# sruckh/echo-tts

Measured on AMD Instinct MI355X. Metric: audio-sec/sec/GPU @ seq_len=640, 40 steps, CFG(text=3, spk=8); 1/2/4/8 GPU, higher is better.
Workload: dtype bf16; 1 GPU; C2: 48 utterance(s)/step/GPU (24 per sampler call, 2 HIP stream(s)), seq_len=640, 40 Euler steps (20 CFG x3 rows + 20 x1 row), cfg_text=3.0 cfg_spk=8.0, text 436 tokens padded to 768, one speaker latent (1,2560,80) encoded per call and shared by its rows, EchoDiT bf16 + Fish S1-DAC decode fp32, random weights; parallelism=dp1 (independent utterances, weight broadcast only)

## Files before the change

### echo-tts_amd/_lib.py

```python
from __future__ import annotations

import ctypes as C
import os

HERE = os.path.dirname(os.path.abspath(__file__))
LIB_PATH = os.environ.get("ECHO_LIB_PATH") or os.path.join(HERE, "libechohip.so")

ECHO_F32, ECHO_BF16 = 0, 1
ABI_VERSION = 8

c_i64 = C.c_int64
vp = C.c_void_p


class EchoConfig(C.Structure):
    _fields_ = [
        ("precision", C.c_int),
        ("latent_size", C.c_int), ("model_size", C.c_int), ("num_layers", C.c_int), ("num_heads", C.c_int),
        ("intermediate_size", C.c_int),
        ("norm_eps", C.c_float),
        ("text_vocab_size", C.c_int), ("text_model_size", C.c_int), ("text_num_layers", C.c_int),
        ("text_num_heads", C.c_int), ("text_intermediate_size", C.c_int),
        ("speaker_patch_size", C.c_int), ("speaker_model_size", C.c_int), ("speaker_num_layers", C.c_int),
        ("speaker_num_heads", C.c_int), ("speaker_intermediate_size", C.c_int),
# ... 71 lines not shown


SIGNATURES = {
    "echo_abi_version": (C.c_int, []),
    "echo_last_error": (C.c_char_p, [vp]),
    "echo_ctx_create": (C.c_int, [C.POINTER(EchoConfig), C.c_int, C.POINTER(vp)]),
    "echo_ctx_destroy": (None, [vp]),
    "echo_load_tensor": (C.c_int, [vp, C.c_char_p, vp, C.c_int, C.c_int, C.POINTER(c_i64), C.c_int]),
    "echo_finalize_dit": (C.c_int, [vp, vp]),
    "echo_finalize_dac": (C.c_int, [vp, vp]),
    "echo_set_rope_table": (C.c_int, [vp, vp, C.c_int]),
    "echo_set_ae_rope_table": (C.c_int, [vp, vp, C.c_int]),
    "echo_encode_text": (C.c_int, [vp, vp, vp, C.POINTER(C.c_int32), C.c_int, C.c_int, vp]),
    "echo_encode_speaker": (C.c_int, [vp, vp, vp, C.POINTER(C.c_int32), C.c_int, C.c_int, vp]),
    "echo_encode_latent_prefix": (C.c_int, [vp, vp, C.c_int, C.c_int, C.c_long, vp]),
    "echo_scale_speaker_kv": (C.c_int, [vp, C.c_float, C.c_int, vp]),
    "echo_dit_forward": (C.c_int, [vp, vp, vp, C.c_int, C.c_int, C.c_int, C.c_int, C.c_int, C.POINTER(C.c_int32),
                                   C.POINTER(C.c_int32), vp, vp]),
    "echo_dit_forward_t": (C.c_int, [vp, vp, vp, C.c_int, C.POINTER(C.c_int32), C.c_int, C.c_int, C.c_int, C.c_int, C.c_int,
                                     C.POINTER(C.c_int32), C.POINTER(C.c_int32), vp, vp]),
    "echo_sample_euler": (C.c_int, [vp, C.POINTER(EchoSamplerParams), vp, vp, vp]),
    "echo_dac_decode": (C.c_int, [vp, vp, C.c_int, C.c_float, vp, vp]),
    "echo_dac_decode_zq": (C.c_int, [vp, vp, C.c_int, vp, vp]),
    "echo_dac_decode_batch": (C.c_int, [vp, vp, C.c_int, C.c_int, C.c_float, vp, c_i64, vp]),
    "echo_set_pca": (C.c_int, [vp, vp, vp, C.c_int, vp]),
    "echo_dac_hop": (C.c_int, [vp]),
    "echo_finalize_dac_encoder": (C.c_int, [vp, vp]),
    "echo_dac_encode": (C.c_int, [vp, vp, C.c_long, vp, vp, vp, vp]),
    "echo_set_pca_encode": (C.c_int, [vp, vp, vp, C.c_float, C.c_int, vp]),
    "echo_op_gemm": (C.c_int, [C.c_int, C.POINTER(EchoGemmDesc), vp]),
    "echo_op_quant_rows_fp8": (C.c_int, [vp, c_i64, vp, c_i64, vp, C.c_int, C.c_int, vp]),
    "echo_op_norm_adaln_fp8": (C.c_int, [vp, c_i64, vp, c_i64, vp, C.c_int, C.c_int, C.c_float, vp, vp, vp]),
    "echo_op_presplit_weights": (C.c_int, [vp, c_i64, c_i64, vp]),
    "echo_op_pack_rows": (C.c_int, [vp, C.c_int, c_i64, vp, C.c_int, c_i64, C.c_int, C.c_int, C.c_int, C.c_int, vp]),
    "echo_op_attention_bf16": (C.c_int, [C.POINTER(EchoAttnDesc), vp]),
    "echo_op_attention_bf16_len": (C.c_int, [C.POINTER(EchoAttnDesc), vp, vp]),
    "echo_op_norm": (C.c_int, [C.c_int, C.c_int, vp, c_i64, vp, c_i64, C.c_int, C.c_int, C.c_float, vp, vp, vp]),
    "echo_op_headnorm_rope": (C.c_int, [C.c_int, vp, c_i64, c_i64, C.c_int, C.c_int, C.c_int, C.c_int, vp, c_i64, C.c_float,
                                        C.c_int, C.c_int, vp, C.c_int, C.c_int, vp]),
    "echo_op_transpose_heads": (C.c_int, [C.c_int, vp, c_i64, vp, c_i64, c_i64, C.c_int, C.c_int, C.c_int, C.c_int, vp]),
    "echo_debug_get_kv": (C.c_int, [vp, C.c_int, C.c_int, vp, vp, C.POINTER(C.c_int), C.POINTER(C.c_int)]),
    "echo_debug_corrupt_tile": (C.c_int, [vp, C.c_int]),
    "echo_op_resample": (C.c_int, [vp, c_i64, vp, C.c_int, C.c_int, C.c_int, C.c_int, vp, c_i64, vp]),
    "echo_voice_capture": (C.c_int, [vp, C.POINTER(vp), vp]),
    "echo_voice_bind": (C.c_int, [vp, vp, vp]),
    "echo_sample_euler_items": (C.c_int, [vp, C.POINTER(EchoSamplerParams), C.POINTER(EchoSamplerItem), vp, vp, vp]),
    "echo_dit_forward_pos": (C.c_int, [vp, vp, vp, C.c_int, C.POINTER(C.c_int32), C.c_int, C.c_int, C.c_int, C.POINTER(C.c_int32), C.c_int,
                                       C.POINTER(C.c_int32), C.POINTER(C.c_int32), vp, vp]),
    "echo_sample_euler_items_pos": (C.c_int, [vp, C.POINTER(EchoSamplerParams), C.POINTER(EchoSamplerItem), C.POINTER(C.c_int32), vp, vp, vp]),
    "echo_dit_forward_len": (C.c_int, [vp, vp, vp, C.c_int, C.POINTER(C.c_int32), C.c_int, C.c_int, C.c_int, C.POINTER(C.c_int32),
                                       C.POINTER(C.c_int32), C.c_int, C.POINTER(C.c_int32), C.POINTER(C.c_int32), vp, vp]),
    "echo_sample_euler_items_len": (C.c_int, [vp, C.POINTER(EchoSamplerParams), C.POINTER(EchoSamplerItem), C.POINTER(C.c_int32),
                                              C.POINTER(C.c_int32), vp, vp, vp]),
    "echo_scale_speaker_kv_items": (C.c_int, [vp, C.POINTER(C.c_float), C.POINTER(C.c_int32), C.c_int, vp]),
    "echo_voice_bind_items": (C.c_int, [vp, C.POINTER(vp), C.c_int, vp]),
    "echo_voice_bytes": (c_i64, [vp]),
    "echo_voice_destroy": (None, [vp]),
    "echo_dac_decode_tail": (C.c_int, [vp, vp, C.c_int, C.c_int, C.c_float, vp, vp]),
    "echo_workspace_bytes": (c_i64, [vp]),
    "echo_fp8_calibrate": (C.c_int, [vp, C.c_int]),
    "echo_fp8_calibration": (C.c_int, [vp, C.POINTER(C.c_float), C.c_int]),
    "echo_fp8_set_static_scales": (C.c_int, [vp, C.POINTER(C.c_float), C.c_int]),
    "echo_reserve_workspace": (C.c_int, [vp, C.c_int, C.c_int, C.c_int, C.c_int, C.c_int]),
    "echo_op_find_flattening_point": (C.c_int, [vp, c_i64, C.c_int, C.c_int, C.c_int, C.c_int, C.c_float, C.c_float, vp, vp]),
    "echo_op_trailing_quiet": (C.c_int, [C.POINTER(vp), C.POINTER(c_i64), C.c_int, C.c_int, C.c_float, vp, vp]),
    "echo_op_assemble_chunks": (C.c_int, [C.POINTER(vp), C.POINTER(c_i64), C.POINTER(c_i64), C.POINTER(c_i64), C.POINTER(C.c_int32),
# ... 37 lines not shown
```

### echo-tts_amd/build.py

```python
from __future__ import annotations

import os
import shutil
import subprocess
import sys

HERE = os.path.dirname(os.path.abspath(__file__))
CSRC = os.path.join(HERE, "csrc")
LIB = os.path.join(HERE, "libechohip.so")
SOURCES = ["gemm_pp.hip", "gemm.hip", "gemm_f32.hip", "attention.hip", "elementwise.hip", "dac.hip", "postproc.hip", "engine.hip"]
EXTRA_FLAGS = {"attention.hip": ["-fno-slp-vectorize"]}
COMMON_FLAGS = ["-ffp-contract=off"]


def _hipcc() -> str:
    for c in (os.environ.get("HIPCC"), "/opt/rocm/bin/hipcc", shutil.which("hipcc")):
        if c and os.path.exists(c):
            return c
    raise RuntimeError("hipcc not found (ROCm toolchain required)")


def needs_build() -> bool:
    if not os.path.exists(LIB):
        return True
    t = os.path.getmtime(LIB)
    deps = [os.path.join(CSRC, f) for f in os.listdir(CSRC)] + [os.path.join(HERE, "..", "include", "echo_hip.h")]
    return any(os.path.getmtime(d) > t for d in deps)


def build(force: bool = False, verbose: bool = True) -> str:
    if not force and not needs_build():
        return LIB
    objs = []
    os.makedirs(os.path.join(HERE, "build"), exist_ok=True)
    procs = []
    for src in SOURCES:
        obj = os.path.join(HERE, "build", src.replace(".hip", ".o"))
        cmd = [_hipcc(), "--offload-arch=gfx950", "-O3", "-std=c++17", "-fPIC"] + COMMON_FLAGS + EXTRA_FLAGS.get(src, []) + ["-c", os.path.join(CSRC, src), "-o", obj]
        procs.append((src, subprocess.Popen(cmd, stdout=subprocess.PIPE, stderr=subprocess.STDOUT, text=True)))
        objs.append(obj)
    for src, p in procs:
        out, _ = p.communicate()
        if p.returncode != 0:
# ... 13 lines not shown
```

### echo-tts_amd/csrc/common.h

```cpp
#pragma once
#include <hip/hip_runtime.h>
#include <stdint.h>
#include <string.h>
#include <atomic>
#include <string>

inline hipError_t ensure_dyn_lds(const void* kern, int bytes, std::atomic<unsigned long long>& done) {
  int dev = 0;
  hipError_t e = hipGetDevice(&dev);
  if (e != hipSuccess) return e;
  const unsigned long long bit = 1ull << (dev & 63);
  if (done.load(std::memory_order_acquire) & bit) return hipSuccess;
  e = hipFuncSetAttribute(kern, hipFuncAttributeMaxDynamicSharedMemorySize, bytes);
  if (e == hipSuccess) done.fetch_or(bit, std::memory_order_release);
  return e;
}

typedef uint16_t bf16_t;
typedef __attribute__((ext_vector_type(8))) short bf16x8;
typedef __attribute__((ext_vector_type(4))) short bf16x4;
typedef __attribute__((ext_vector_type(4))) float f32x4;
typedef __attribute__((ext_vector_type(4))) int i32x4;
typedef __attribute__((ext_vector_type(8))) int i32x8;
typedef __attribute__((ext_vector_type(16))) float f32x16;
// ... 74 lines not shown
  int nbatch, nbi;
  long a_bo, a_bi, w_bo, w_bi, c_bo, c_bi;
  float acc_scale;
  const void* bias; long bias_bo, bias_bi; int vec_mod;
  float div;
  int act;
  const void* colscale;
  const void* res; long ldres, res_bo, res_bi;
  const void* snake_alpha;
  int store_main;
  int swiglu;
  int cfg;
  int ksplit;
  void* ws; long ws_bytes;
  int split3;
  int w_presplit;
  float a_scale_const;
  void* c8; long c8_ld; float c8_inv;
  int pp_gn;
  int snake_fast;
  void* sink;
  int qkv_mode, qkv_D, qkv_S, rope_heads, pos0;
  int qkv_gate_act;
  float qk_eps;
  int rope_mod;
  const void* qk_w; const void* rope;
  void* vt; long vt_ld, vt_row_stride;
  int fp8; const float* a_scale; const float* w_scale;
};
int gemm_tile_m(int cfg);
int gemm_num_cfgs();
void gemm_args_init(GemmArgs* g);
template <typename T> hipError_t launch_gemm_nt(const GemmArgs& g, hipStream_t st);

struct AttnSeg {
  const bf16_t* K; long k_ld, k_row_stride, k_head_stride;
  const bf16_t* Vt; long vt_ld, vt_row_stride, vt_head_stride;
  const int* nkeys;
  const float* bias; long bias_row_stride;
  int kv_mod;
};
struct AttnArgs {
  const bf16_t* Q; long q_ld, q_row_stride;
  bf16_t* O; long o_ld, o_row_stride;
  const bf16_t* G; long g_ld, g_row_stride;
  int g_act;
  int S, H, rows;
  int nseg; AttnSeg seg[4];
  int causal;
  float scale;
  void* prof;
  int* redo;
  const int* redo_filter;
  int q_block0;
  int redo_nb;
  int q128;
  uint8_t* O8; long o8_ld, o8_row_stride; float o8_inv;
  const int* qlen;
};
inline long attn_redo_words(int rows, int H, int S) { return (long)rows * H * ((S + 127) / 128); }
hipError_t launch_attention_bf16(const AttnArgs& a, hipStream_t st);

enum NormMode { NORM_ADALN = 0, NORM_RMS_W = 1, NORM_AE_RMS = 2, NORM_LAYER = 3 };
template <typename T>
hipError_t launch_norm(int mode, const T* x, long ldx, T* y, long ldy, int rows, int D, float eps,
                       const T* w0, const T* w1, hipStream_t st);
// ... 106 lines not shown
```

### echo-tts_amd/csrc/engine.hip

```cpp
#include "common.h"
#include "../../include/echo_hip.h"

#include <dlfcn.h>

#include <cmath>
#include <cstdio>
#include <cstdlib>
#include <map>
#include <memory>
#include <mutex>
#include <string>
#include <vector>

namespace {

thread_local std::string g_create_error;

struct Plan { int cfg = 0, ksplit = 1; };
std::map<int, std::map<std::vector<long>, Plan>> g_plans;
std::mutex g_plans_mu;

inline long rup(long x, long m) { return (x + m - 1) / m * m; }

std::string plan_file_path() {
// ... 1762 lines not shown
        for (auto& ru : Bk.ru) {
          CK(launch_presplit_w(ru.w7, rup(Bk.co, 128), 7L * Bk.co, st));
          CK(launch_presplit_w(ru.w1, rup(Bk.co, 128), Bk.co, st));
        }
      }
    }
    }
    CK(hipStreamSynchronize(st));
    drop_raw({"quantizer.", "decoder."});
    dac_ready = true;
    return ECHO_OK;
  }

  bool dac_split3 = getenv("ECHO_DAC_EXACT_FP32") ? atoi(getenv("ECHO_DAC_EXACT_FP32")) == 0 : true;
  bool dac_fast_sin = getenv("ECHO_DAC_FAST_SIN") ? atoi(getenv("ECHO_DAC_FAST_SIN")) != 0 : true;
  DevBuf b_sink;
  template <typename X>
  int frun(const GemmArgs& g_in, hipStream_t st) {
    GemmArgs g = g_in;
    g.split3 = sizeof(X) == 4 && dac_split3 ? 1 : 0;
    if (sizeof(X) == 2) g.w_presplit = 0;
    if (!b_sink.p) CK(b_sink.reserve(262144));
    g.sink = b_sink.p;
    g.snake_fast = dac_fast_sin ? 1 : 0;
    if constexpr (sizeof(X) == 2) {
      const bool big = (long)g.M * g.Npad >= 256L * 256 * 64;
      g.cfg = !big ? 0 : g.N % 192 == 0 && g.N % 256 != 0 ? 8 : g.N % 96 == 0 && g.N % 128 != 0 ? 9 : g.N % 256 > 0 && g.N % 256 <= 128 ? 3 : 2;
      g.ksplit = 1;
    } else {
      CKI(plan_gemm<X>(g, st));
    }
    return run_planned<X>(g, st, false);
  }
  template <typename X>
  static GemmArgs FG(const X* A, long lda, const X* W, long ldw, X* C, long ldc, long M, int N, int K) {
    GemmArgs g;
    gemm_args_init(&g);
    g.A = A; g.lda = lda; g.W = W; g.ldw = ldw; g.C = C; g.ldc = ldc; g.M = (int)M; g.N = N; g.K = K;
    g.Npad = (int)rup(N, 128);
    return g;
  }

  int set_pca(const float* w, const float* mean, int on_device, hipStream_t st) override {
    if (!dac_ready) return fail("echo_finalize_dac was not called");
    const int C = cfg.dac_latent_dim, Lz = cfg.latent_size;
    const hipMemcpyKind kind = on_device ? hipMemcpyDeviceToDevice : hipMemcpyHostToDevice;
    CK(hipMemcpy2DAsync(pca_w, pca_kpad * sizeof(float), w, Lz * sizeof(float), Lz * sizeof(float), C, kind, st));
    CK(hipMemcpyAsync(pca_b, mean, C * sizeof(float), kind, st));
    CK(hipStreamSynchronize(st));
    pca_set = true;
    return ECHO_OK;
  }
  bool pca_set = false;
  int dac_decode(const float* lat, int Tn, float latent_scale, float* wav, hipStream_t st) override {
    if (!pca_set) return fail("echo_set_pca was not called");
    return dac_run(lat, nullptr, Tn, latent_scale, wav, st);
  }
  int dac_decode_zq(const float* z, int Tn, float* wav, hipStream_t st) override { return dac_run(nullptr, z, Tn, 1.0f, wav, st); }
  int dac_decode_tail(const float* lat, int Tn, int f0, float latent_scale, float* wav, hipStream_t st) override {
    if (!pca_set) return fail("echo_set_pca was not called");
    if (f0 < 0 || f0 >= Tn) return fail("bad first frame");
    return dac_run(lat, nullptr, Tn, latent_scale, wav, st, f0);
  }

  template <typename X>
  int dac_transformer(std::vector<DacLayerT<X>>& layers, X* x, int Tn, int C, int nh, int hd, int ff, int window, X* xn_buf,
// ... 380 lines not shown
    if (!front)
    for (auto& U : dups) {
      { GemmArgs g = FG(cur, C, U.w, C, other, (long)U.f * C, rows, U.f * C, C); g.bias = U.b; g.vec_mod = C; CKI(frun<T>(g, st)); }
      rows *= U.f;
      CK(launch_dwconv_ln(other, C, cur, C, (int)rows, (int)rows, C, U.dw, U.db, U.lnw, U.lnb, 1e-6f, st));
      { GemmArgs g = FG(cur, C, U.p1w, C, third, 4L * C, rows, 4 * C, C); g.bias = U.p1b; g.act = 2; CKI(frun<T>(g, st)); }
      { GemmArgs g = FG(third, 4L * C, U.p2w, 4L * C, other, C, rows, C, 4 * C); g.bias = U.p2b; g.colscale = U.gamma; g.res = other; g.ldres = C; CKI(frun<T>(g, st)); }
      std::swap(cur, other);
    }
    T *Y = other, *S = third, *Uu = nullptr;
    {
      const int ch = cpad(cfg.dac_decoder_dim);
      GemmArgs g = FG(cur, C, dconv0_w, 7L * C, Y, ch, rows, ch, C);
      g.w_presplit = !DAC_BF16 && dac_split3;
      g.taps = 7; g.tap_base = -6; g.tap_shift = 1; g.bias = dconv0_b;
      g.store_main = 0; g.C2 = S; g.snake_alpha = dblocks[0].alpha;
      CKI(frun<T>(g, st));
      Uu = cur;
    }
    for (size_t bi = 0; bi < dblocks.size(); ++bi) {
      DacBlock& Bk = dblocks[bi];
      {
        GemmArgs g = FG(S, Bk.ci, Bk.wt, 2L * Bk.ci, Y, (long)Bk.r * Bk.co, rows, Bk.r * Bk.co, Bk.ci);
        g.w_presplit = !DAC_BF16 && dac_split3;
        g.taps = 2; g.tap_base = -1; g.tap_shift = 1; g.bias = Bk.bt; g.vec_mod = Bk.co;
        g.C2 = Uu; g.snake_alpha = Bk.ru[0].a0;
        CKI(frun<T>(g, st));
        rows *= Bk.r;
        std::swap(S, Uu);
      }
      const int dil[3] = {1, 3, 9};
      for (int j = 0; j < 3; ++j) {
        DacRU& ru = Bk.ru[j];
        {
          GemmArgs g = FG(S, Bk.co, ru.w7, 7L * Bk.co, Uu, Bk.co, rows, Bk.co, Bk.co);
          g.w_presplit = !DAC_BF16 && dac_split3;
          g.taps = 7; g.tap_base = -6 * dil[j]; g.tap_shift = dil[j]; g.bias = ru.b7;
          g.store_main = 0; g.C2 = Uu; g.snake_alpha = ru.a1;
          CKI(frun<T>(g, st));
        }
        {
          const T* next_alpha = j < 2 ? Bk.ru[j + 1].a0 : (bi + 1 < dblocks.size() ? dblocks[bi + 1].alpha : dfinal_alpha);
          GemmArgs g = FG(Uu, Bk.co, ru.w1, Bk.co, Y, Bk.co, rows, Bk.co, Bk.co);
          g.w_presplit = !DAC_BF16 && dac_split3;
          g.bias = ru.b1; g.res = Y; g.ldres = Bk.co;
          g.store_main = j < 2 ? 1 : 0; g.C2 = S; g.snake_alpha = next_alpha;
          CKI(frun<T>(g, st));
        }
      }
    }
    const int cl = cpad(cfg.dac_decoder_dim >> cfg.dac_n_rates);
    CK(launch_conv_out_tanh(S, cl, wav, rows, (int)rows, cl, 7, dout_w, dout_b, st));
    if (profiling) {
      CK(hipEventRecord(ev[2], st));
      CK(hipEventSynchronize(ev[2]));
      CK(hipEventElapsedTime(&prof.ms_total, ev[0], ev[2]));
      prof.ms_mod = 0.f; prof.ms_steps = prof.ms_total;
      collect_gemm_times();
    }
    return ECHO_OK;
  }
};

__global__ void add_seg_bias_kernel(float* __restrict__ dst, long ld, int rows, int off, int w, const float* __restrict__ bias, long bias_ld,
                                    int kv_mod) {
  const long i = (long)blockIdx.x * blockDim.x + threadIdx.x;
// ... 213 lines not shown
}

int echo_op_norm_adaln_fp8(const void* x, int64_t ldx, void* q, int64_t ldq, float* scale, int rows, int D, float eps,
                           const void* scale1p, const void* shift, void* stream) {
  if (D < 8 || (D & 7) || D > 4096 || rows < 1) return ECHO_ERR;
  return op_status(launch_norm_adaln_fp8(x, ldx, q, ldq, scale, rows, D, eps, scale1p, shift, (hipStream_t)stream));
}

int echo_op_gemm(int dtype, const echo_gemm_desc* d, void* stream) {
  GemmArgs g;
  gemm_args_init(&g);
  g.A = d->A; g.W = d->W; g.C = d->C; g.C2 = d->C2; g.M = d->M; g.N = d->N; g.K = d->K; g.Npad = d->Npad;
  g.lda = d->lda; g.ldw = d->ldw; g.ldc = d->ldc; g.taps = d->taps < 1 ? 1 : d->taps; g.tap_base = d->tap_base; g.tap_shift = d->tap_shift;
  g.nbatch = d->nbatch < 1 ? 1 : d->nbatch; g.nbi = d->nbi < 1 ? 1 : d->nbi;
  g.a_bo = d->a_bo; g.a_bi = d->a_bi; g.w_bo = d->w_bo; g.w_bi = d->w_bi; g.c_bo = d->c_bo; g.c_bi = d->c_bi;
  g.acc_scale = d->acc_scale == 0.0f ? 1.0f : d->acc_scale;
  g.bias = d->bias; g.bias_bo = d->bias_bo; g.bias_bi = d->bias_bi; g.vec_mod = d->vec_mod; g.div = d->div; g.act = d->act;
  g.colscale = d->colscale; g.res = d->res; g.ldres = d->ldres; g.res_bo = d->res_bo; g.res_bi = d->res_bi;
  g.snake_alpha = d->snake_alpha; g.store_main = d->store_main; g.swiglu = d->swiglu;
  g.cfg = d->cfg; g.ksplit = d->ksplit; g.ws = d->ws; g.ws_bytes = d->ws_bytes; g.split3 = d->split3; g.w_presplit = d->split3 ? d->w_presplit : 0;
  g.fp8 = d->fp8; g.a_scale = d->a_scale; g.w_scale = d->w_scale;
  g.a_scale_const = d->a_scale_const; g.c8 = d->c8; g.c8_ld = d->c8_ld; g.c8_inv = d->c8_inv; g.qkv_gate_act = d->qkv_gate_act;
  g.qkv_mode = d->qkv_mode; g.qkv_D = d->qkv_D; g.qkv_S = d->qkv_S; g.rope_mod = d->qkv_S; g.rope_heads = d->rope_heads; g.pos0 = d->pos0; g.qk_eps = d->qk_eps;
  g.qk_w = d->qk_w; g.rope = d->rope; g.vt = d->vt; g.vt_ld = d->vt_ld; g.vt_row_stride = d->vt_row_stride;
  if (dtype == ECHO_BF16 && g.snake_alpha && g.C2) {
    static thread_local DevBuf sink_buf[64];
    int dev = 0; (void)hipGetDevice(&dev);
    DevBuf& sb = sink_buf[dev & 63];
    if (hipError_t e = sb.reserve(262144); e != hipSuccess) return op_status(e);
    g.sink = sb.p;
  }
  return op_status(dtype == ECHO_BF16 ? launch_gemm_nt<bf16_t>(g, (hipStream_t)stream) : launch_gemm_nt<float>(g, (hipStream_t)stream));
}
int echo_op_presplit_weights(float* w, int64_t rows, int64_t ld, void* stream) {
  return op_status(launch_presplit_w(w, rows, ld, (hipStream_t)stream));
}
int echo_op_pack_rows(const void* src, int sdt, int64_t sld, void* dst, int ddt, int64_t dld, int rows, int cols, int dst_row0,
                      int swiglu_half, void* stream) {
  return op_status(launch_pack_rows(src, sdt, sld, dst, ddt, dld, rows, cols, dst_row0, swiglu_half, (hipStream_t)stream));
}
static int op_attention_bf16(const echo_attn_desc* d, const int32_t* qlen, void* stream) {
  AttnArgs a;
  memset(&a, 0, sizeof(a));
  a.qlen = qlen;
  a.Q = (const bf16_t*)d->Q; a.q_ld = d->q_ld; a.q_row_stride = d->q_row_stride;
  a.O = (bf16_t*)d->O; a.o_ld = d->o_ld; a.o_row_stride = d->o_row_stride;
  a.G = (const bf16_t*)d->G; a.g_ld = d->g_ld; a.g_row_stride = d->g_row_stride;
  a.S = d->S; a.H = d->H; a.rows = d->rows; a.nseg = d->nseg; a.causal = d->causal; a.scale = d->scale; a.prof = d->prof;
  a.O8 = (uint8_t*)d->O8; a.o8_ld = d->o8_ld; a.o8_row_stride = d->o8_row_stride; a.o8_inv = d->o8_inv; a.g_act = d->g_activated;
  for (int s = 0; s < d->nseg && s < 4; ++s) {
    a.seg[s].K = (const bf16_t*)d->seg[s].K; a.seg[s].k_ld = d->seg[s].k_ld; a.seg[s].k_row_stride = d->seg[s].k_row_stride;
    a.seg[s].k_head_stride = d->seg[s].k_head_stride;
    a.seg[s].Vt = (const bf16_t*)d->seg[s].Vt; a.seg[s].vt_ld = d->seg[s].vt_ld; a.seg[s].vt_row_stride = d->seg[s].vt_row_stride;
    a.seg[s].vt_head_stride = d->seg[s].vt_head_stride;
    a.seg[s].nkeys = d->seg[s].nkeys; a.seg[s].bias = d->seg[s].bias; a.seg[s].bias_row_stride = d->seg[s].bias_row_stride;
    a.seg[s].kv_mod = d->seg[s].kv_mod;
  }
  a.redo = (int*)d->redo;
  if (!a.redo && a.rows > 0 && a.H > 0 && a.S > 0) {
    static thread_local DevBuf redo_buf[64];
    int dev = 0; (void)hipGetDevice(&dev);
    DevBuf& rb = redo_buf[dev & 63];
    if (hipError_t e = rb.reserve((size_t)attn_redo_words(a.rows, a.H, a.S) * sizeof(int)); e != hipSuccess) return op_status(e);
    a.redo = rb.as<int>();
  }
  return op_status(launch_attention_bf16(a, (hipStream_t)stream));
// ... 56 lines not shown
```

### include/echo_hip.h

```cpp
#ifndef ECHO_HIP_H
#define ECHO_HIP_H
#include <stdint.h>
#ifdef __cplusplus
extern "C" {
#endif

#define ECHO_F32 0
#define ECHO_BF16 1
#define ECHO_ABI_VERSION 8

typedef struct echo_ctx echo_ctx;

typedef struct {
  int precision;
  int latent_size, model_size, num_layers, num_heads, intermediate_size;
  float norm_eps;
  int text_vocab_size, text_model_size, text_num_layers, text_num_heads, text_intermediate_size;
  int speaker_patch_size, speaker_model_size, speaker_num_layers, speaker_num_heads, speaker_intermediate_size;
  int timestep_embed_size, adaln_rank;
  int has_latent_encoder;
  int dac_latent_dim, dac_decoder_dim, dac_n_rates, dac_rates[8];
  int dac_post_layers, dac_post_heads, dac_post_head_dim, dac_post_ffn, dac_post_window;
  int dac_n_up, dac_up_factors[4];
  float dac_norm_eps;
// ... 93 lines not shown
int echo_dac_decode_batch(echo_ctx* ctx, const float* latent, int B, int T, float latent_scale, float* wav_out, int64_t wav_stride, void* stream);
int echo_dac_decode_tail(echo_ctx* ctx, const float* latent, int T, int first_frame, float latent_scale, float* wav_out, void* stream);
int echo_set_pca(echo_ctx* ctx, const float* w, const float* mean, int on_device, void* stream);
int echo_dac_hop(echo_ctx* ctx);
int echo_dac_encode(echo_ctx* ctx, const float* audio, long n_samples, float* latent_out, int32_t* codes_out, float* zq_out,
                    void* stream);
int echo_set_pca_encode(echo_ctx* ctx, const float* w, const float* bias, float scale, int on_device, void* stream);

typedef struct {
  const void* A; const void* W; void* C; void* C2;
  int M, N, K, Npad; int64_t lda, ldw, ldc;
  int taps, tap_base, tap_shift;
  int nbatch, nbi; int64_t a_bo, a_bi, w_bo, w_bi, c_bo, c_bi;
  float acc_scale;
  const void* bias; int64_t bias_bo, bias_bi; int vec_mod;
  float div; int act;
  const void* colscale;
  const void* res; int64_t ldres, res_bo, res_bi;
  const void* snake_alpha;
  int store_main, swiglu;
  int cfg;
  int ksplit; void* ws; int64_t ws_bytes;
  int split3;
  int fp8;
  const float* a_scale; const float* w_scale;
  int qkv_mode, qkv_D, qkv_S, rope_heads, pos0; float qk_eps;
  const void* qk_w; const void* rope; void* vt; int64_t vt_ld, vt_row_stride;
  int w_presplit;
  float a_scale_const; void* c8; int64_t c8_ld; float c8_inv;
  int qkv_gate_act;
} echo_gemm_desc;
int echo_op_gemm(int dtype, const echo_gemm_desc* d, void* stream);
int echo_op_presplit_weights(float* w, int64_t rows, int64_t ld, void* stream);
int echo_op_quant_rows_fp8(const void* x, int64_t ldx, void* q, int64_t ldq, float* scale, int rows, int K, void* stream);
int echo_op_norm_adaln_fp8(const void* x, int64_t ldx, void* q, int64_t ldq, float* scale, int rows, int D, float eps,
                           const void* scale1p, const void* shift, void* stream);
int echo_op_pack_rows(const void* src, int src_dtype, int64_t src_ld, void* dst, int dst_dtype, int64_t dst_ld, int rows,
                      int cols, int dst_row0, int swiglu_half, void* stream);

typedef struct {
  const void* K; int64_t k_ld, k_row_stride, k_head_stride;
  const void* Vt; int64_t vt_ld, vt_row_stride, vt_head_stride;
  const int32_t* nkeys; const float* bias; int64_t bias_row_stride; int kv_mod;
} echo_attn_seg;
typedef struct {
  const void* Q; int64_t q_ld, q_row_stride;
  void* O; int64_t o_ld, o_row_stride;
  const void* G; int64_t g_ld, g_row_stride;
  int S, H, rows, nseg; echo_attn_seg seg[4]; int causal; float scale;
  void* prof;
  void* redo;
  void* O8; int64_t o8_ld, o8_row_stride; float o8_inv;
  int g_activated;
} echo_attn_desc;
int echo_op_attention_bf16(const echo_attn_desc* d, void* stream);
int echo_op_attention_bf16_len(const echo_attn_desc* d, const int32_t* qlen_dev, void* stream);

int echo_op_norm(int dtype, int mode, const void* x, int64_t ldx, void* y, int64_t ldy, int rows, int D, float eps,
                 const void* w0, const void* w1, void* stream);
int echo_op_headnorm_rope(int dtype, void* x, int64_t ldx, int64_t t_stride, int nt, int rows, int S, int H, const void* w,
                          int64_t w_stride, float eps, int do_norm, int rope_heads, const void* rope, int pos0, int pos_mul,
                          void* stream);
int echo_op_transpose_heads(int dtype, const void* v, int64_t ldv, void* vt, int64_t vt_ld, int64_t vt_b_stride, int B, int S,
                            int H, int HD, void* stream);

int echo_op_find_flattening_point(const float* latent, int64_t item_stride, int B, int T, int W, int window, float target,
// ... 28 lines not shown
```

Before: 202.5 audio-s/s (whole job; divide by n_gpus for per-GPU).

## Fuse DAC residual unit conv7+snake+conv1 into one kernel for C=96

Adds a dedicated HIP kernel that computes the DAC decoder residual unit's dilated 7-tap conv, bias, Snake activation and the 1x1 conv in one pass. The intermediate activation stays in registers and is fed into the second MFMA chain, with W1 streamed through the same LDS ring. This removes one GEMM launch and the global-memory round trip of the intermediate tensor. It only applies to 96-channel blocks on the fp32 split3 path, is on by default behind ECHO_DAC_FUSE_RU, and keeps a second accumulator set live, which raises register pressure.

After: 203.0 audio-s/s (whole job; divide by n_gpus for per-GPU), median of 6. About the same (+0.3%).

```diff
diff --git a/echo-tts_amd/_lib.py b/echo-tts_amd/_lib.py
--- a/echo-tts_amd/_lib.py
+++ b/echo-tts_amd/_lib.py
@@ -127,6 +127,7 @@
     "echo_op_quant_rows_fp8": (C.c_int, [vp, c_i64, vp, c_i64, vp, C.c_int, C.c_int, vp]),
     "echo_op_norm_adaln_fp8": (C.c_int, [vp, c_i64, vp, c_i64, vp, C.c_int, C.c_int, C.c_float, vp, vp, vp]),
     "echo_op_presplit_weights": (C.c_int, [vp, c_i64, c_i64, vp]),
+    "echo_op_dac_resunit": (C.c_int, [vp, vp, vp, vp, vp, vp, vp, vp, vp, vp, c_i64, C.c_int, C.c_int, C.c_int, vp]),
     "echo_op_pack_rows": (C.c_int, [vp, C.c_int, c_i64, vp, C.c_int, c_i64, C.c_int, C.c_int, C.c_int, C.c_int, vp]),
     "echo_op_attention_bf16": (C.c_int, [C.POINTER(EchoAttnDesc), vp]),
     "echo_op_attention_bf16_len": (C.c_int, [C.POINTER(EchoAttnDesc), vp, vp]),
diff --git a/echo-tts_amd/build.py b/echo-tts_amd/build.py
--- a/echo-tts_amd/build.py
+++ b/echo-tts_amd/build.py
@@ -8,7 +8,7 @@
 HERE = os.path.dirname(os.path.abspath(__file__))
 CSRC = os.path.join(HERE, "csrc")
 LIB = os.path.join(HERE, "libechohip.so")
-SOURCES = ["gemm_pp.hip", "gemm.hip", "gemm_f32.hip", "attention.hip", "elementwise.hip", "dac.hip", "postproc.hip", "engine.hip"]
+SOURCES = ["gemm_pp.hip", "gemm.hip", "gemm_f32.hip", "dac_resunit.hip", "attention.hip", "elementwise.hip", "dac.hip", "postproc.hip", "engine.hip"]
 EXTRA_FLAGS = {"attention.hip": ["-fno-slp-vectorize"]}
 COMMON_FLAGS = ["-ffp-contract=off"]
 
diff --git a/echo-tts_amd/csrc/common.h b/echo-tts_amd/csrc/common.h
--- a/echo-tts_amd/csrc/common.h
+++ b/echo-tts_amd/csrc/common.h
@@ -130,6 +130,8 @@
 int gemm_num_cfgs();
 void gemm_args_init(GemmArgs* g);
 template <typename T> hipError_t launch_gemm_nt(const GemmArgs& g, hipStream_t st);
+bool dac_resunit_fused(int C);
+hipError_t launch_dac_resunit(const GemmArgs& g, const float* b7, const float* a1, const float* w1, hipStream_t st);
 
 struct AttnSeg {
   const bf16_t* K; long k_ld, k_row_stride, k_head_stride;
diff --git a/echo-tts_amd/csrc/dac_resunit.hip b/echo-tts_amd/csrc/dac_resunit.hip
--- /dev/null
+++ b/echo-tts_amd/csrc/dac_resunit.hip
@@ -0,0 +1,240 @@
+#include "gemm_tile.h"
+
+namespace {
+
+template <int C_>
+struct RuCfg {
+  static constexpr int C = C_, BM = 128, BN = C_, NW = 4, NT = 256, TN = C_ / 32;
+  static constexpr int STAGE_BYTES = (BM + BN) * KBYTES, STAGES = 2, RING = STAGES * STAGE_BYTES;
+  static constexpr int VEC_BYTES = 3 * C_ * 4;
+  static constexpr int SMEM = RING + VEC_BYTES;
+  static constexpr int PIECES = (BM + BN) / 8, PPW = PIECES / NW;
+  static_assert(PIECES % NW == 0, "pieces must divide evenly over the waves");
+  static_assert(32 * BN * 4 <= RING, "epilogue slab must fit");
+};
+
+template <int C, int NTAIL>
+__global__ void __launch_bounds__(256, 2) dac_resunit_kernel(const GemmArgs p, const float* __restrict__ b7, const float* __restrict__ a1,
+                                                             const float* __restrict__ W1) {
+  typedef RuCfg<C> CF;
+  extern __shared__ __attribute__((aligned(16))) char smem[];
+  constexpr int BM = CF::BM, TN = CF::TN, PPW = CF::PPW, STAGES = CF::STAGES, KE = KBYTES / 4;
+  const int tid = threadIdx.x, lane = tid & 63;
+  const int wid = __builtin_amdgcn_readfirstlane(tid >> 6);
+  const int tiles_m = (p.M + BM - 1) / BM;
+  int bid = blockIdx.x;
+  {
+    const int q = tiles_m >> 3, r = tiles_m & 7, xcd = bid & 7, idx = bid >> 3;
+    bid = (xcd < r ? xcd * (q + 1) : r * (q + 1) + (xcd - r) * q) + idx;
+  }
+  const int tile_m = bid;
+
+  float* vec = (float*)(smem + CF::RING);
+  if (tid < C) {
+    const float al = a1[tid];
+    vec[tid] = b7[tid];
+    vec[C + tid] = al;
+    vec[2 * C + tid] = 1.0f / (al + 1e-9f);
+  }
+  asm volatile("s_waitcnt lgkmcnt(0)" ::: "memory");
+
+  constexpr int kb_per_tap = C / KE;
+  const int nk1 = kb_per_tap * p.taps;
+  const int nk = nk1 + kb_per_tap;
+
+  const char* src[PPW];
+  int w1o[PPW];
+  bool is_a[PPW];
+#pragma unroll
+  for (int i = 0; i < PPW; ++i) {
+    const int piece = wid * PPW + i;
+    const int r = piece * 8 + (lane >> 3);
+    const int chunk = (lane & 7) ^ ((r >> 1) & 7);
+    is_a[i] = piece * 8 < BM;
+    w1o[i] = 0;
+    if (is_a[i]) {
+      int gm = tile_m * BM + r;
+      gm = gm < p.M ? gm : p.M - 1;
+      src[i] = (const char*)p.A + (long)(gm + p.tap_base) * p.lda * 4L + chunk * 16;
+    } else {
+      const int gn = r - BM;
+      src[i] = (const char*)p.W + (long)gn * p.ldw * 4L + chunk * 16;
+      w1o[i] = gn * C * 4 + chunk * 16;
+    }
+  }
+  const long a_tap_bytes = ((long)p.tap_shift * p.lda - (long)C) * 4L;
+  int kb = 0;
+  long a_off = 0, w_off = 0;
+  int w1_off = 0;
+
+  const char* nsrc[PPW];
+  char* ndst = nullptr;
+  auto next_src = [&](int slot, bool w1step) {
+    ndst = smem + slot * CF::STAGE_BYTES + wid * (PPW * 1024);
+    if (!w1step) {
+#pragma unroll
+      for (int i = 0; i < PPW; ++i) nsrc[i] = src[i] + (is_a[i] ? a_off : w_off);
+      a_off += KBYTES; w_off += KBYTES;
+      if (++kb == kb_per_tap) { kb = 0; a_off += a_tap_bytes; }
+    } else {
+#pragma unroll
+      for (int i = 0; i < PPW; ++i) nsrc[i] = (const char*)W1 + (w1o[i] + w1_off);
+      w1_off += KBYTES;
+    }
+  };
+
+  const int fr = lane & 31, fh = lane >> 5;
+  const int sw = (lane >> 1) & 7;
+  const int a_row0 = (wid * 32 + fr) * KBYTES;
+  const int w_row0 = (BM + fr) * KBYTES;
+
+  f32x16 acc[TN], acc2[TN];
+#pragma unroll
+  for (int i = 0; i < TN; ++i)
+#pragma unroll
+    for (int r = 0; r < 16; ++r) { acc[i][r] = 0.0f; acc2[i][r] = 0.0f; }
+
+  {
+    next_src(0, false);
+#pragma unroll
+    for (int i = 0; i < PPW; ++i) glds16(nsrc[i], ndst + i * 1024);
+  }
+  int issued = 1;
+
+  constexpr int NMF = 16 * TN;
+  auto mfma_step = [&](f32x16 (&d)[TN], const bf16x8 (&whi)[TN], const bf16x8 (&wlo)[TN], const bf16x8& ahi, const bf16x8& alo, int& mf, int& piece,
+                       bool more, bool w1step) __attribute__((always_inline)) {
+#pragma unroll
+    for (int tn = 0; tn < TN; ++tn) {
+      d[tn] = __builtin_amdgcn_mfma_f32_32x32x16_bf16(wlo[tn], ahi, d[tn], 0, 0, 0);
+      d[tn] = __builtin_amdgcn_mfma_f32_32x32x16_bf16(whi[tn], alo, d[tn], 0, 0, 0);
+      d[tn] = __builtin_amdgcn_mfma_f32_32x32x16_bf16(whi[tn], ahi, d[tn], 0, 0, 0);
+      mf += 8;
+#pragma unroll
+      for (int due = 0; due < PPW; ++due) {
+        if (piece < PPW && mf * PPW * DMA_SPREAD_DEN >= (piece + 1) * NMF) {
+          if (more && !(w1step && is_a[piece])) glds16(nsrc[piece], ndst + piece * 1024);
+          ++piece;
+          __builtin_amdgcn_sched_barrier(0);
+        }
+      }
+    }
+  };
+  auto load_w = [&](const char* sa, int kk, bf16x8 (&whi)[TN], bf16x8 (&wlo)[TN]) __attribute__((always_inline)) {
+#pragma unroll
+    for (int t = 0; t < TN; ++t) {
+      const char* rowp = sa + w_row0 + t * 32 * KBYTES;
+      whi[t] = *(const bf16x8*)(rowp + (((2 * kk + fh) ^ sw) << 4));
+      wlo[t] = *(const bf16x8*)(rowp + (((4 + 2 * kk + fh) ^ sw) << 4));
+    }
+  };
+  auto split8 = [&](const f32x8& x, bf16x8& hi, bf16x8& lo) __attribute__((always_inline)) {
+    const hbf16x8 h = __builtin_convertvector(x, hbf16x8);
+    const f32x8 hf = __builtin_convertvector(h, f32x8);
+    const hbf16x8 l = __builtin_convertvector(x - hf, hbf16x8);
+    hi = __builtin_bit_cast(bf16x8, h);
+    lo = __builtin_bit_cast(bf16x8, l);
+  };
+
+  for (int it = 0; it < nk1; ++it) {
+    wait_vmcnt<0>();
+    __builtin_amdgcn_s_barrier();
+    const bool w1step = issued >= nk1;
+    next_src((it + 1) % STAGES, w1step); ++issued;
+    const char* sa = smem + (it % STAGES) * CF::STAGE_BYTES;
+    int mf = 0, piece = 0;
+#pragma unroll
+    for (int kk = 0; kk < 2; ++kk) {
+      bf16x8 whi[TN], wlo[TN], ahi, alo;
+      load_w(sa, kk, whi, wlo);
+      {
+        const char* rowp = sa + a_row0;
+        const f32x4 x0 = *(const f32x4*)(rowp + (((4 * kk + 2 * fh) ^ sw) << 4));
+        const f32x4 x1 = *(const f32x4*)(rowp + (((4 * kk + 2 * fh + 1) ^ sw) << 4));
+        f32x8 x;
+#pragma unroll
+        for (int i = 0; i < 4; ++i) { x[i] = x0[i]; x[4 + i] = x1[i]; }
+        split8(x, ahi, alo);
+      }
+      mfma_step(acc, whi, wlo, ahi, alo, mf, piece, true, w1step);
+    }
+  }
+
+  const bool fast = p.snake_fast != 0;
+#pragma unroll
+  for (int j = 0; j < TN; ++j) {
+    const int it = nk1 + j;
+    wait_vmcnt<0>();
+    __builtin_amdgcn_s_barrier();
+    const bool more = issued < nk;
+    if (more) { next_src((it + 1) % STAGES, true); ++issued; }
+    const char* sa = smem + (it % STAGES) * CF::STAGE_BYTES;
+    float u[16];
+#pragma unroll
+    for (int g = 0; g < 4; ++g) {
+      const int c0 = 32 * j + 8 * g + 4 * fh;
+      const f32x4 bb = *(const f32x4*)(vec + c0), al = *(const f32x4*)(vec + C + c0), ial = *(const f32x4*)(vec + 2 * C + c0);
+#pragma unroll
+      for (int i = 0; i < 4; ++i) {
+        const float y = acc[j][4 * g + i] + bb[i];
+        const float sn = fast ? sin_fast(al[i] * y) : sinf(al[i] * y);
+        u[4 * g + i] = y + ial[i] * (sn * sn);
+      }
+    }
+    int mf = 0, piece = 0;
+#pragma unroll
+    for (int kk = 0; kk < 2; ++kk) {
+      bf16x8 whi[TN], wlo[TN], ahi, alo;
+      load_w(sa, kk, whi, wlo);
+      f32x8 x;
+#pragma unroll
+      for (int i = 0; i < 4; ++i) {
+        const float lo_g = u[8 * kk + i], hi_g = u[8 * kk + 4 + i];
+        const float got = __shfl_xor(fh ? lo_g : hi_g, 32, 64);
+        x[i] = fh ? got : lo_g;
+        x[4 + i] = fh ? hi_g : got;
+      }
+      split8(x, ahi, alo);
+      mfma_step(acc2, whi, wlo, ahi, alo, mf, piece, more, true);
+    }
+  }
+
+  const int fr_ = fr, fh_ = fh;
+  gemm_epilogue<float, false, BM, C, CF::NT, true, false, NTAIL>(p, (float*)smem, tid, tile_m, 0, tiles_m, 0, 0, 0L, 0, [&](int pass, float* slab) {
+    constexpr int CPR = C / 4;
+    if (wid == pass) {
+#pragma unroll
+      for (int tn = 0; tn < TN; ++tn)
+#pragma unroll
+        for (int g = 0; g < 4; ++g) {
+          const int chunk = tn * 8 + 2 * g + fh_;
+          f32x4 v;
+          v[0] = acc2[tn][4 * g]; v[1] = acc2[tn][4 * g + 1]; v[2] = acc2[tn][4 * g + 2]; v[3] = acc2[tn][4 * g + 3];
+          *(f32x4*)(slab + slab_pos<CPR>(fr_, chunk) * 4) = v;
+        }
+    }
+  });
+}
+
+template <int C, int NTAIL>
+hipError_t launch_ru(const GemmArgs& g, const float* b7, const float* a1, const float* w1, hipStream_t st) {
+  typedef RuCfg<C> CF;
+  static std::atomic<unsigned long long> prepared{0};
+  auto kern = dac_resunit_kernel<C, NTAIL>;
+  if (hipError_t e = ensure_dyn_lds((const void*)kern, CF::SMEM, prepared); e != hipSuccess) return e;
+  hipLaunchKernelGGL(kern, dim3((g.M + CF::BM - 1) / CF::BM), dim3(CF::NT), CF::SMEM, st, g, b7, a1, w1);
+  return hipGetLastError();
+}
+
+}
+
+bool dac_resunit_fused(int C) { return C == 96; }
+
+hipError_t launch_dac_resunit(const GemmArgs& g, const float* b7, const float* a1, const float* w1, hipStream_t st) {
+  if (!dac_resunit_fused(g.N) || g.K != g.N || g.M <= 0 || g.taps != 7 || g.tap_shift < 1 || g.tap_base != -6 * g.tap_shift || !g.split3 ||
+      !g.w_presplit || g.nbatch != 1 || g.ksplit > 1 || !g.A || !g.W || !g.C || !g.C2 || g.A == g.C2 || !g.res || !g.bias || !g.snake_alpha ||
+      !g.sink || !b7 || !a1 || !w1 || g.lda != g.N || g.ldc != g.N || g.ldres != g.N || g.ldw != 7L * g.N || g.vec_mod || g.acc_scale != 1.0f ||
+      g.div != 0.0f || g.act || g.colscale)
+    return hipErrorInvalidValue;
+  return g.store_main ? launch_ru<96, 5>(g, b7, a1, w1, st) : launch_ru<96, 3>(g, b7, a1, w1, st);
+}
diff --git a/echo-tts_amd/csrc/engine.hip b/echo-tts_amd/csrc/engine.hip
--- a/echo-tts_amd/csrc/engine.hip
+++ b/echo-tts_amd/csrc/engine.hip
@@ -1818,6 +1818,33 @@
     }
     return run_planned<X>(g, st, false);
   }
+  bool dac_fuse_ru = getenv("ECHO_DAC_FUSE_RU") ? atoi(getenv("ECHO_DAC_FUSE_RU")) != 0 : true;
+  int frun_resunit(const GemmArgs& g_in, const float* b7, const float* a1, const float* w1, hipStream_t st) {
+    GemmArgs g = g_in;
+    g.split3 = 1; g.w_presplit = 1; g.cfg = 0; g.ksplit = 1;
+    if (!b_sink.p) CK(b_sink.reserve(262144));
+    g.sink = b_sink.p;
+    g.snake_fast = dac_fast_sin ? 1 : 0;
+    if (profiling) {
+      if (gemm_events_used == gemm_events.size()) {
+        hipEvent_t a, b;
+        CK(hipEventCreate(&a)); CK(hipEventCreate(&b));
+        gemm_events.emplace_back(a, b);
+      }
+      if (gemm_event_flops.size() < gemm_events.size()) gemm_event_flops.resize(gemm_events.size(), 0.0);
+      if (gemm_event_shape.size() < gemm_events.size()) gemm_event_shape.resize(gemm_events.size());
+      const size_t slot = gemm_events_used++;
+      auto& e = gemm_events[slot];
+      CK(hipEventRecord(e.first, st));
+      CK(launch_dac_resunit(g, b7, a1, w1, st));
+      CK(hipEventRecord(e.second, st));
+      gemm_event_flops[slot] = 0.0;
+      gemm_event_shape[slot] = {g.M, g.N, g.K, 8 , 0, 0, 0, 70 , 1, 1};
+      return ECHO_OK;
+    }
+    CK(launch_dac_resunit(g, b7, a1, w1, st));
+    return ECHO_OK;
+  }
   template <typename X>
   static GemmArgs FG(const X* A, long lda, const X* W, long ldw, X* C, long ldc, long M, int N, int K) {
     GemmArgs g;
@@ -2264,6 +2291,18 @@
       const int dil[3] = {1, 3, 9};
       for (int j = 0; j < 3; ++j) {
         DacRU& ru = Bk.ru[j];
+        if constexpr (!DAC_BF16) {
+          if (dac_fuse_ru && dac_split3 && dac_resunit_fused(Bk.co)) {
+            const T* next_alpha = j < 2 ? Bk.ru[j + 1].a0 : (bi + 1 < dblocks.size() ? dblocks[bi + 1].alpha : dfinal_alpha);
+            GemmArgs g = FG(S, Bk.co, ru.w7, 7L * Bk.co, Y, Bk.co, rows, Bk.co, Bk.co);
+            g.taps = 7; g.tap_base = -6 * dil[j]; g.tap_shift = dil[j];
+            g.bias = ru.b1; g.res = Y; g.ldres = Bk.co;
+            g.store_main = j < 2 ? 1 : 0; g.C2 = Uu; g.snake_alpha = next_alpha;
+            CKI(frun_resunit(g, ru.b7, ru.a1, ru.w1, st));
+            std::swap(S, Uu);
+            continue;
+          }
+        }
         {
           GemmArgs g = FG(S, Bk.co, ru.w7, 7L * Bk.co, Uu, Bk.co, rows, Bk.co, Bk.co);
           g.w_presplit = !DAC_BF16 && dac_split3;
@@ -2543,6 +2582,34 @@
   }
   return op_status(dtype == ECHO_BF16 ? launch_gemm_nt<bf16_t>(g, (hipStream_t)stream) : launch_gemm_nt<float>(g, (hipStream_t)stream));
 }
+int echo_op_dac_resunit(const float* s, const float* res, float* y, float* s_out, const float* w7, const float* b7, const float* a1,
+                        const float* w1, const float* b1, const float* next_alpha, int64_t rows, int C, int dil, int store_main, void* stream) {
+  if (!s || !res || !s_out || (store_main && !y) || !w7 || !b7 || !a1 || !w1 || !b1 || !next_alpha || rows < 1 || rows > 0x7fffffffL || C < 32 ||
+      C % 32 || dil < 1 || s == s_out) {
+    g_create_error = "echo_op_dac_resunit: bad argument";
+    return ECHO_ERR;
+  }
+  static thread_local DevBuf sink_buf[64];
+  int dev = 0; (void)hipGetDevice(&dev);
+  DevBuf& sb = sink_buf[dev & 63];
+  if (hipError_t e = sb.reserve(262144); e != hipSuccess) return op_status(e);
+  hipStream_t st = (hipStream_t)stream;
+  GemmArgs g7, g1;
+  gemm_args_init(&g7);
+  g7.A = s; g7.lda = C; g7.W = w7; g7.ldw = 7L * C; g7.C = s_out; g7.C2 = s_out; g7.ldc = C; g7.M = (int)rows; g7.N = C; g7.K = C;
+  g7.Npad = (C + 127) / 128 * 128; g7.taps = 7; g7.tap_base = -6 * dil; g7.tap_shift = dil; g7.bias = b7; g7.store_main = 0; g7.snake_alpha = a1;
+  g7.split3 = 1; g7.w_presplit = 1; g7.sink = sb.p; g7.cfg = C % 192 == 0 ? 6 : C % 96 == 0 ? 7 : 0;
+  g1 = g7;
+  g1.taps = 1; g1.tap_base = 0; g1.tap_shift = 0; g1.W = w1; g1.ldw = C; g1.bias = b1; g1.res = res; g1.ldres = C;
+  g1.C = y ? (void*)y : (void*)s_out; g1.store_main = store_main ? 1 : 0; g1.snake_alpha = next_alpha;
+  if (dac_resunit_fused(C)) {
+    g1.A = s; g1.W = w7; g1.ldw = 7L * C; g1.taps = 7; g1.tap_base = -6 * dil; g1.tap_shift = dil;
+    return op_status(launch_dac_resunit(g1, b7, a1, w1, st));
+  }
+  if (hipError_t e = launch_gemm_nt<float>(g7, st); e != hipSuccess) return op_status(e);
+  g1.A = s_out;
+  return op_status(launch_gemm_nt<float>(g1, st));
+}
 int echo_op_presplit_weights(float* w, int64_t rows, int64_t ld, void* stream) {
   return op_status(launch_presplit_w(w, rows, ld, (hipStream_t)stream));
 }
diff --git a/include/echo_hip.h b/include/echo_hip.h
--- a/include/echo_hip.h
+++ b/include/echo_hip.h
@@ -149,6 +149,8 @@
 } echo_gemm_desc;
 int echo_op_gemm(int dtype, const echo_gemm_desc* d, void* stream);
 int echo_op_presplit_weights(float* w, int64_t rows, int64_t ld, void* stream);
+int echo_op_dac_resunit(const float* s, const float* res, float* y, float* s_out, const float* w7, const float* b7, const float* a1,
+                        const float* w1, const float* b1, const float* next_alpha, int64_t rows, int C, int dil, int store_main, void* stream);
 int echo_op_quant_rows_fp8(const void* x, int64_t ldx, void* q, int64_t ldq, float* scale, int rows, int K, void* stream);
 int echo_op_norm_adaln_fp8(const void* x, int64_t ldx, void* q, int64_t ldq, float* scale, int rows, int D, float eps,
                            const void* scale1p, const void* shift, void* stream);
```
